# intel-aero/aero-optical-flow

Measured on AMD Instinct MI355X. Metric: frame-pairs/s (640x480, 8x8 SAD, +-4 search), higher is better.
Workload: dtype u8

## Files before the change

aero-optical-flow_amd/csrc/aof_device.hpp:

```cpp
#pragma once

#include <hip/hip_runtime.h>

#include <cstdint>

#include "aof_internal.hpp"

namespace aof {

typedef unsigned long long u64;
typedef uint32_t u32x2 __attribute__((ext_vector_type(2)));
typedef uint32_t u32x4 __attribute__((ext_vector_type(4)));

constexpr int kRawBuffer = 0x00020000;

__device__ __forceinline__ uint32_t fast_div(uint32_t n, FastDiv d) { return (__umulhi(n, d.mul) + n) >> d.shift; }

__device__ __forceinline__ int equalise_delta(const uint32_t *sums, int64_t pair, int level,
                                              uint32_t npix)
{
    if (!sums) return 0;
    const uint32_t sp = sums[pair * 4 + 0 * 2 + level];
    const uint32_t sc = sums[pair * 4 + 1 * 2 + level];
    const int mp = (int)((sp + npix / 2) / npix);
    const int mc = (int)((sc + npix / 2) / npix);
    return mp - mc;
}

__device__ __forceinline__ int clamp_u8(int v) { return v < 0 ? 0 : (v > 255 ? 255 : v); }

typedef unsigned short ushort2_t __attribute__((ext_vector_type(2)));

__device__ __forceinline__ uint32_t sat_delta_u16x2(int delta)
{
    const uint32_t m = (uint32_t)(delta < 0 ? -delta : delta);
    return (m << 8) | (m << 24);
}

template <bool NEG>
__device__ __forceinline__ uint32_t sat_shift_u8x4(uint32_t v, uint32_t d8)
{
    const ushort2_t odd = __builtin_bit_cast(ushort2_t, v), even = __builtin_bit_cast(ushort2_t, v << 8);
    const ushort2_t d = __builtin_bit_cast(ushort2_t, d8);
    const ushort2_t o2 = NEG ? __builtin_elementwise_sub_sat(odd, d) : __builtin_elementwise_add_sat(odd, d);
    const ushort2_t e2 = NEG ? __builtin_elementwise_sub_sat(even, d) : __builtin_elementwise_add_sat(even, d);
    return __builtin_amdgcn_perm(__builtin_bit_cast(uint32_t, o2), __builtin_bit_cast(uint32_t, e2),
                                 0x07030501u);
}

__device__ __forceinline__ uint32_t sat_add_u8x4(uint32_t v, int delta)
{
    const uint32_t d8 = sat_delta_u16x2(delta);
    return delta < 0 ? sat_shift_u8x4<true>(v, d8) : sat_shift_u8x4<false>(v, d8);
}

__device__ __forceinline__ uint4 sat_add_u8x16(uint4 v, int delta)
{
    const uint32_t d8 = sat_delta_u16x2(delta);
    if (delta < 0) {
        v.x = sat_shift_u8x4<true>(v.x, d8); v.y = sat_shift_u8x4<true>(v.y, d8);
        v.z = sat_shift_u8x4<true>(v.z, d8); v.w = sat_shift_u8x4<true>(v.w, d8);
    } else {
        v.x = sat_shift_u8x4<false>(v.x, d8); v.y = sat_shift_u8x4<false>(v.y, d8);
        v.z = sat_shift_u8x4<false>(v.z, d8); v.w = sat_shift_u8x4<false>(v.w, d8);
    }
    return v;
}

__device__ __forceinline__ uint32_t box2(uint32_t a, uint32_t b)
{
    const uint32_t m = 0x00FF00FFu;
    const uint32_t s = (a & m) + ((a >> 8) & m) + (b & m) + ((b >> 8) & m) + 0x00020002u;
    return (s >> 2) & m;
}

__device__ __forceinline__ uint32_t byte_sum(uint32_t w, uint32_t acc)
{
    return __builtin_amdgcn_sad_u8(w, 0u, acc);
}

__device__ __forceinline__ uint32_t wave_min_u32(uint32_t v)
{
#pragma unroll
    for (int o = 32; o >= 1; o >>= 1) {
        const uint32_t other = (uint32_t)__shfl_xor((int)v, o, 64);
        v = other < v ? other : v;
    }
    return v;
}

__device__ __forceinline__ uint32_t wave_sum_u32(uint32_t v)
{
#pragma unroll
    for (int o = 32; o >= 1; o >>= 1) v += (uint32_t)__shfl_xor((int)v, o, 64);
    return v;
}

__device__ __forceinline__ void wave_vote(uint32_t *hist, int bin, bool active)
{
    unsigned long long todo = __ballot(active);
    while (todo) {
        const int leader = __ffsll((long long)todo) - 1;
        const int b = __shfl(bin, leader, 64);
        const unsigned long long same = __ballot(active && bin == b) & todo;
        if ((int)(threadIdx.x & 63) == leader) atomicAdd(&hist[b], (uint32_t)__popcll(same));
        todo &= ~same;
    }
}

__device__ __forceinline__ void wave_vote2(uint32_t *hist_x, uint32_t *hist_y, int bin_x, int bin_y, bool active)
{
    const unsigned long long todo = __ballot(active);
    if (todo == 0) return;
    const int key = bin_x | (bin_y << 16);
    const int leader = __ffsll((long long)todo) - 1;
    const int k = __shfl(key, leader, 64);
    if ((__ballot(active && key == k) & todo) == todo) {
        if ((int)(threadIdx.x & 63) == leader) {
            const uint32_t c = (uint32_t)__popcll(todo);
            atomicAdd(&hist_x[k & 0xFFFF], c);
            atomicAdd(&hist_y[k >> 16], c);
        }
        return;
    }
    wave_vote(hist_x, bin_x, active);
    wave_vote(hist_y, bin_y, active);
}

__device__ __forceinline__ void wave_vote_weighted(uint32_t *hist, int bin, int weight, unsigned long long m1, unsigned long long m2,
                                                   unsigned long long m3, unsigned long long m4)
{
    unsigned long long todo = m1 | m2 | m3 | m4;
    while (todo) {
        const int leader = __ffsll((long long)todo) - 1;
        const int b = __shfl(bin, leader, 64);
        const unsigned long long same = __ballot(weight != 0 && bin == b) & todo;
        const uint32_t total = (uint32_t)(__popcll(same & m1) + 2 * __popcll(same & m2) + 3 * __popcll(same & m3) + 4 * __popcll(same & m4));
        if ((int)(threadIdx.x & 63) == leader) atomicAdd(&hist[b], total);
        todo &= ~same;
    }
}

__device__ __forceinline__ void wave_vote2_weighted(uint32_t *hist_x, uint32_t *hist_y, int key, int weight)
{
    const unsigned long long m1 = __ballot(weight == 1), m2 = __ballot(weight == 2), m3 = __ballot(weight == 3), m4 = __ballot(weight == 4);
    const unsigned long long todo = m1 | m2 | m3 | m4;
    if (todo == 0) return;
    const int leader = __ffsll((long long)todo) - 1;
    const int k = __shfl(key, leader, 64);
    if ((__ballot(weight != 0 && key == k) & todo) == todo) {
        if ((int)(threadIdx.x & 63) == leader) {
            const uint32_t total = (uint32_t)(__popcll(m1) + 2 * __popcll(m2) + 3 * __popcll(m3) + 4 * __popcll(m4));
            atomicAdd(&hist_x[k & 0xFFFF], total);
            atomicAdd(&hist_y[k >> 16], total);
        }
        return;
    }
    wave_vote_weighted(hist_x, key & 0xFFFF, weight, m1, m2, m3, m4);
    wave_vote_weighted(hist_y, key >> 16, weight, m1, m2, m3, m4);
}

__device__ __forceinline__ uint32_t xcd_remap(uint32_t b, uint32_t total)
{
    const uint32_t q = total / 8, r = total % 8, xcd = b % 8, slot = b / 8;
    const uint32_t base = xcd < r ? xcd * (q + 1) : r * (q + 1) + (xcd - r) * q;
    return base + slot;
}

}
```

aero-optical-flow_amd/csrc/aof_reduce.hpp:

```cpp
#pragma once

#include "aof_device.hpp"
#include "aof_internal.hpp"

namespace aof {

__device__ __forceinline__ void peak_window(int pos, int n, int *lo, int *hi)
{
    *lo = *hi = pos;
    if (pos > 1 && pos < n - 2) { *lo = pos - 2; *hi = pos + 2; }
    else if (pos == 0) { *hi = pos + 2; }
    else if (pos == n - 1) { *lo = pos - 2; }
    else if (pos == 1) { *lo = pos - 1; *hi = pos + 2; }
    else if (pos == n - 2) { *lo = pos - 2; *hi = pos + 1; }
}

template <typename T>
__device__ __forceinline__ T floor_div(T a, T b)
{
    T q = a / b;
    if ((a % b) < 0) q--;
    return q;
}

__device__ __forceinline__ void write_flow(const FlowTail &a, int64_t pair, int n, uint32_t vx, uint32_t wx, uint32_t vy,
                                           uint32_t wy, const int *sums)
{
#pragma clang fp contract(off)
    const int centre = 2 * a.range + 1;
    aof_flow out;
    out.flow_x = out.flow_y = 0.0f;
    out.count = (uint32_t)sums[2];
    out.quality = 0;
    out.flags = 0;
    out.pred_x = out.pred_y = 0;
    int px = 0, py = 0;
    const long long count = sums[2];
    const bool small = (long long)n * a.nblocks < (1ll << 28);
    if (count > (long long)a.min_valid && count > 0) {
        if (a.hist_filter) {
            out.flow_x = (__fdiv_rn((float)vx, (float)wx) - (float)centre) / 2.0f;
            out.flow_y = (__fdiv_rn((float)vy, (float)wy) - (float)centre) / 2.0f;
            if (small) {
                px = floor_div<int>((int)(2 * vx + wx), (int)(2 * wx)) - centre;
                py = floor_div<int>((int)(2 * vy + wy), (int)(2 * wy)) - centre;
            } else {
                px = (int)(floor_div<long long>(2ll * vx + wx, 2ll * wx) - centre);
                py = (int)(floor_div<long long>(2ll * vy + wy, 2ll * wy) - centre);
            }
        } else {
            out.flow_x = __fdiv_rn((float)sums[0] * 0.5f, (float)count);
            out.flow_y = __fdiv_rn((float)sums[1] * 0.5f, (float)count);
            if (small) {
                px = floor_div<int>(2 * sums[0] + (int)count, 2 * (int)count);
                py = floor_div<int>(2 * sums[1] + (int)count, 2 * (int)count);
            } else {
                px = (int)floor_div<long long>(2ll * sums[0] + count, 2ll * count);
                py = (int)floor_div<long long>(2ll * sums[1] + count, 2ll * count);
            }
        }
        out.quality = small ? (uint8_t)((uint32_t)count * 255u / (uint32_t)a.nblocks)
                            : (uint8_t)((unsigned long long)count * 255ull / (unsigned long long)a.nblocks);
        out.flags |= AOF_FLAG_FLOW_VALID;
    }
    if (a.emit_predictor) {
        out.pred_x = (int8_t)px;
        out.pred_y = (int8_t)py;
    } else if (a.pred) {
        const aof_flow p = a.pred[pair];
        out.pred_x = p.pred_x;
        out.pred_y = p.pred_y;
        if (p.flags & AOF_FLAG_FLOW_VALID) out.flags |= AOF_FLAG_PRED_VALID;
    }
    a.flows[pair] = out;
}

__device__ __forceinline__ void finalise_flow_wave_bins(const FlowTail &a, int64_t pair, uint32_t hx, uint32_t hy,
                                                        int sum2x, int sum2y, int total, aof_flow *record_out = nullptr,
                                                        const aof_flow *pred_rec = nullptr);

__device__ __forceinline__ void finalise_flow_wave(const FlowTail &a, int64_t pair, const uint32_t *hist_x,
                                                   const uint32_t *hist_y, const int *sums, aof_flow *record_out = nullptr,
                                                   const aof_flow *pred_rec = nullptr)
{
    const int n = 2 * (2 * a.range + 1) + 1;
    const int k = (int)(threadIdx.x & 63);
    finalise_flow_wave_bins(a, pair, k < n ? hist_x[k] : 0u, k < n ? hist_y[k] : 0u, sums[0], sums[1], sums[2],
                            record_out, pred_rec);
}

__device__ __forceinline__ void finalise_flow_wave_bins(const FlowTail &a, int64_t pair, uint32_t hx, uint32_t hy,
                                                        int sum2x, int sum2y, int total, aof_flow *record_out,
                                                        const aof_flow *pred_rec)
{
    const int centre = 2 * a.range + 1, n = 2 * centre + 1;
    const int k = (int)(threadIdx.x & 63);
    const int sums[3] = {sum2x, sum2y, total};
    uint32_t mx = hx, my = hy;
#pragma unroll
    for (int o = 32; o >= 1; o >>= 1) {
        const uint32_t ox = (uint32_t)__shfl_xor((int)mx, o, 64), oy = (uint32_t)__shfl_xor((int)my, o, 64);
        mx = ox > mx ? ox : mx;
        my = oy > my ? oy : my;
    }
    const int posx = __ffsll((long long)__ballot(k < n && hx == mx)) - 1;
    const int posy = __ffsll((long long)__ballot(k < n && hy == my)) - 1;
    int lox, hix, loy, hiy;
    peak_window(posx, n, &lox, &hix);
    peak_window(posy, n, &loy, &hiy);
    const bool inx = k >= lox && k <= hix, iny = k >= loy && k <= hiy;
    const uint32_t vx = wave_sum_u32(inx ? (uint32_t)k * hx : 0u), wx = wave_sum_u32(inx ? hx : 0u);
    const uint32_t vy = wave_sum_u32(iny ? (uint32_t)k * hy : 0u), wy = wave_sum_u32(iny ? hy : 0u);
    const bool axis_y = k == 1;
    const uint32_t v = axis_y ? vy : vx, w = axis_y ? wy : wx;
    const int s2 = axis_y ? sums[1] : sums[0];
    const long long count = sums[2];
    const bool valid = count > (long long)a.min_valid && count > 0;
    const bool small = (long long)n * a.nblocks < (1ll << 28);
    float flow = 0.0f;
    int pred = 0;
    if (k < 2 && valid) {
#pragma clang fp contract(off)
        if (a.hist_filter) {
            flow = (__fdiv_rn((float)v, (float)w) - (float)centre) / 2.0f;
            if (a.emit_predictor)
                pred = small ? floor_div<int>((int)(2 * v + w), (int)(2 * w)) - centre
                             : (int)(floor_div<long long>(2ll * v + w, 2ll * w) - centre);
        } else {
            flow = __fdiv_rn((float)s2 * 0.5f, (float)count);
            if (a.emit_predictor)
                pred = small ? floor_div<int>(2 * s2 + (int)count, 2 * (int)count)
                             : (int)floor_div<long long>(2ll * s2 + count, 2ll * count);
        }
    }
    const float flow_y = __shfl(flow, 1, 64);
    const int pred_y = __shfl(pred, 1, 64);
    if (k == 0) {
        aof_flow out;
        out.flow_x = flow; out.flow_y = flow_y;
        out.count = (uint32_t)sums[2];
        out.quality = 0;
        out.flags = 0;
        out.pred_x = out.pred_y = 0;
        if (valid) {
            out.quality = small ? (uint8_t)((uint32_t)count * 255u / (uint32_t)a.nblocks)
                                : (uint8_t)((unsigned long long)count * 255ull / (unsigned long long)a.nblocks);
            out.flags |= AOF_FLAG_FLOW_VALID;
        }
        if (a.emit_predictor) {
            out.pred_x = (int8_t)pred;
            out.pred_y = (int8_t)pred_y;
        } else if (a.pred) {
            const aof_flow p = pred_rec ? *pred_rec : a.pred[pair];
            out.pred_x = p.pred_x;
            out.pred_y = p.pred_y;
            if (p.flags & AOF_FLAG_FLOW_VALID) out.flags |= AOF_FLAG_PRED_VALID;
        }
        a.flows[pair] = out;
        if (record_out) *record_out = out;
    }
}

__device__ __forceinline__ void vote_add_agent(uint32_t *p, uint32_t v)
{
    (void)__hip_atomic_fetch_add(p, v, __ATOMIC_RELAXED, __HIP_MEMORY_SCOPE_AGENT);
}

__device__ __forceinline__ void wave_vote_agent(uint32_t *hist, int bin, bool active)
{
    unsigned long long todo = __ballot(active);
    while (todo) {
        const int leader = __ffsll((long long)todo) - 1;
        const int b = __shfl(bin, leader, 64);
        const unsigned long long same = __ballot(active && bin == b) & todo;
        if ((int)(threadIdx.x & 63) == leader) vote_add_agent(&hist[b], (uint32_t)__popcll(same));
        todo &= ~same;
    }
}

__device__ __forceinline__ void vote_and_arrive(const VoteMem &vm, int range, uint32_t pair, bool member, bool ok,
                                                int bin_x, int bin_y)
{
    const unsigned long long members = __ballot(member);
    if (members == 0) return;
    const int n = 2 * (2 * range + 1) + 1, lane = (int)(threadIdx.x & 63);
    uint32_t *rec = vm.base + (size_t)pair * vm.stride, *hist_x = rec + 2, *hist_y = rec + 2 + n;
    ok = ok && member;
    const unsigned long long voters = __ballot(ok);
    const int head = __ffsll((long long)members) - 1;
    const unsigned long long arrival = ((unsigned long long)__popcll(members) << 32) | (unsigned long long)__popcll(voters);
    bool one_motion = true;
    int k = 0;
    if (voters) {
        const int key = bin_x | (bin_y << 8);
        k = __builtin_amdgcn_readlane(key, __ffsll((long long)voters) - 1);
        one_motion = (__ballot(ok && key == k) & voters) == voters;
    }
    if (one_motion) {
        if (lane == head) {
            if (voters) {
                const uint32_t c = (uint32_t)__popcll(voters);
                vote_add_agent(&hist_x[k & 0xFF], c);
                vote_add_agent(&hist_y[k >> 8], c);
            }
            (void)__hip_atomic_fetch_add(reinterpret_cast<unsigned long long *>(rec), arrival, __ATOMIC_RELAXED,
                                         __HIP_MEMORY_SCOPE_AGENT);
        }
        return;
    }
    wave_vote_agent(hist_x, bin_x, ok);
    wave_vote_agent(hist_y, bin_y, ok);
    if (lane == head)
        (void)__hip_atomic_fetch_add(reinterpret_cast<unsigned long long *>(rec), arrival, __ATOMIC_RELAXED,
                                     __HIP_MEMORY_SCOPE_AGENT);
}

struct NoWalkVotes {
    __device__ __forceinline__ void init() {}
    __device__ __forceinline__ void flush(const VoteMem &, int, uint32_t) {}
    __device__ __forceinline__ void step(const VoteMem &, int, uint32_t, bool, bool, int, int) {}
};
struct WalkVotes {
    int key;
    uint32_t votes, arrivals;

    __device__ __forceinline__ void init() { key = 0; votes = 0; arrivals = 0; }

    __device__ __forceinline__ void flush(const VoteMem &vm, int range, uint32_t pair)
    {
        if (arrivals == 0) return;
        const int n = 2 * (2 * range + 1) + 1;
        uint32_t *rec = vm.base + (size_t)pair * vm.stride, *hist_x = rec + 2, *hist_y = rec + 2 + n;
        if ((threadIdx.x & 63) == 0) {
            if (votes) {
                vote_add_agent(&hist_x[key & 0xFF], votes);
                vote_add_agent(&hist_y[key >> 8], votes);
            }
            (void)__hip_atomic_fetch_add(reinterpret_cast<unsigned long long *>(rec), ((unsigned long long)arrivals << 32) | votes,
                                         __ATOMIC_RELAXED, __HIP_MEMORY_SCOPE_AGENT);
        }
        votes = 0; arrivals = 0;
    }

    __device__ __forceinline__ void step(const VoteMem &vm, int range, uint32_t pair, bool member, bool ok, int bin_x, int bin_y)
    {
        const unsigned long long members = __ballot(member);
        if (members == 0) return;
        ok = ok && member;
        const unsigned long long voters = __ballot(ok);
        const uint32_t nm = (uint32_t)__popcll(members), nv = (uint32_t)__popcll(voters);
        if (voters == 0) { arrivals = (uint32_t)__builtin_amdgcn_readfirstlane((int)(arrivals + nm)); return; }
        const int mine = bin_x | (bin_y << 8);
        const int k = __builtin_amdgcn_readlane(mine, __ffsll((long long)voters) - 1);
        if ((__ballot(ok && mine == k) & voters) == voters) {
            if (votes != 0 && key != k) flush(vm, range, pair);
            key = k;
            votes = (uint32_t)__builtin_amdgcn_readfirstlane((int)(votes + nv));
            arrivals = (uint32_t)__builtin_amdgcn_readfirstlane((int)(arrivals + nm));
            return;
        }
        flush(vm, range, pair);
        const int n = 2 * (2 * range + 1) + 1;
        uint32_t *rec = vm.base + (size_t)pair * vm.stride;
        wave_vote_agent(rec + 2, bin_x, ok);
        wave_vote_agent(rec + 2 + n, bin_y, ok);
        if ((threadIdx.x & 63) == 0)
            (void)__hip_atomic_fetch_add(reinterpret_cast<unsigned long long *>(rec), ((unsigned long long)nm << 32) | nv, __ATOMIC_RELAXED,
                                         __HIP_MEMORY_SCOPE_AGENT);
    }
};

__device__ __forceinline__ void await_votes_and_finalise(const VoteMem &vm, const FlowTail &tail, uint32_t pair)
{
    const uint64_t deadline_ticks = vm.deadline_ticks;
    const int centre = 2 * tail.range + 1, n = 2 * centre + 1, lane = (int)(threadIdx.x & 63);
    uint32_t *rec = vm.base + (size_t)pair * vm.stride, *hist_x = rec + 2, *hist_y = rec + 2 + n;
    const uint64_t t0 = __builtin_amdgcn_s_memrealtime();
    uint32_t hx = 0, hy = 0;
    int total = 0;
    bool complete = false;
    for (;;) {
        uint32_t arrived = 0, announced = 0;
        if (lane < n) {
            hx = __hip_atomic_load(&hist_x[lane], __ATOMIC_RELAXED, __HIP_MEMORY_SCOPE_AGENT);
            hy = __hip_atomic_load(&hist_y[lane], __ATOMIC_RELAXED, __HIP_MEMORY_SCOPE_AGENT);
        } else if (lane == 63) {
            const unsigned long long a = __hip_atomic_load(reinterpret_cast<unsigned long long *>(rec), __ATOMIC_RELAXED,
                                                           __HIP_MEMORY_SCOPE_AGENT);
            arrived = (uint32_t)(a >> 32);
            announced = (uint32_t)a;
        }
        arrived = (uint32_t)__shfl((int)arrived, 63, 64);
        announced = (uint32_t)__shfl((int)announced, 63, 64);
        total = (int)wave_sum_u32(hx);
        complete = arrived == (uint32_t)tail.nblocks && (uint32_t)total == announced && wave_sum_u32(hy) == announced;
        if (complete || __builtin_amdgcn_s_memrealtime() - t0 > deadline_ticks) break;
        __builtin_amdgcn_s_sleep(8);
    }
    if (lane < n) {
        __hip_atomic_store(&hist_x[lane], 0u, __ATOMIC_RELAXED, __HIP_MEMORY_SCOPE_AGENT);
        __hip_atomic_store(&hist_y[lane], 0u, __ATOMIC_RELAXED, __HIP_MEMORY_SCOPE_AGENT);
    } else if (lane == 63) {
        __hip_atomic_store(reinterpret_cast<unsigned long long *>(rec), 0ull, __ATOMIC_RELAXED, __HIP_MEMORY_SCOPE_AGENT);
    }
    if (!complete) {
        if (lane == 0) {
            aof_flow none;
            __builtin_memset(&none, 0, sizeof(none));
            tail.flows[pair] = none;
            __hip_atomic_store(vm.fault, pair + 1u, __ATOMIC_RELEASE, __HIP_MEMORY_SCOPE_SYSTEM);
        }
        return;
    }
    const int sum2x = (int)wave_sum_u32((uint32_t)((lane - centre) * (int)hx));
    const int sum2y = (int)wave_sum_u32((uint32_t)((lane - centre) * (int)hy));
    finalise_flow_wave_bins(tail, (int64_t)pair, hx, hy, sum2x, sum2y, total);
}

__device__ __forceinline__ void finalise_flow(const FlowTail &a, int64_t pair, const uint32_t *hist_x,
                                              const uint32_t *hist_y, const int *sums)
{
    const int centre = 2 * a.range + 1, n = 2 * centre + 1;
    uint32_t vx = 0, wx = 0, vy = 0, wy = 0;
    if (a.hist_filter && sums[2] > a.min_valid && sums[2] > 0) {
        int posx = 0, posy = 0;
        uint32_t maxx = 0, maxy = 0;
        for (int k = 0; k < n; k++) {
            if (hist_x[k] > maxx) { maxx = hist_x[k]; posx = k; }
            if (hist_y[k] > maxy) { maxy = hist_y[k]; posy = k; }
        }
        int lo, hi;
        peak_window(posx, n, &lo, &hi);
        for (int k = lo; k <= hi; k++) { vx += (uint32_t)k * hist_x[k]; wx += hist_x[k]; }
        peak_window(posy, n, &lo, &hi);
        for (int k = lo; k <= hi; k++) { vy += (uint32_t)k * hist_y[k]; wy += hist_y[k]; }
    }
    write_flow(a, pair, n, vx, wx, vy, wy, sums);
}

}
```

aero-optical-flow_amd/csrc/k_reduce.hip:

```cpp
#include "aof_device.hpp"
#include "aof_internal.hpp"
#include "aof_reduce.hpp"

namespace aof {

namespace {

constexpr int kThreads = 256;
constexpr int kMaxHist = 256;
constexpr int64_t kMidPairs = 1024;
constexpr int64_t kWidePairs = 512;

template <int GROUP, int kThreads = 256>
__global__ __launch_bounds__(kThreads) void k_reduce(ReduceArgs a)
{
    constexpr int kGroups = kThreads / GROUP;
    __shared__ uint32_t s_hist[kGroups][2][kMaxHist];
    __shared__ int s_sums[kGroups][3];
    const int grp = (int)threadIdx.x / GROUP, tid = (int)threadIdx.x % GROUP;
    const int64_t pair = (int64_t)blockIdx.x * kGroups + grp;
    if (GROUP < kThreads && pair >= a.n_pairs) return;
    auto sync = [] { if (GROUP == kThreads) __syncthreads(); else __builtin_amdgcn_wave_barrier(); };
    uint32_t (*hist)[kMaxHist] = s_hist[grp];
    int *sums = s_sums[grp];
    const int centre = 2 * a.tail.range + 1, n = 2 * centre + 1;
    for (int k = tid; k < n; k += GROUP) { hist[0][k] = 0; hist[1][k] = 0; }
    if (tid < 3) sums[tid] = 0;
    sync();

    if (a.parts) {
        const uint32_t *parts = a.parts + (size_t)pair * a.nstrips * (size_t)(2 * n);
        for (int k = tid; k < 2 * n; k += GROUP) {
            uint32_t v = 0;
            for (int st = 0; st < a.nstrips; st++) v += parts[(size_t)st * (2 * n) + k];
            const int axis = k >= n, bin = k - axis * n;
            hist[axis][bin] = v;
            if (v) {
                atomicAdd(&sums[axis], (bin - centre) * (int)v);
                if (!axis) atomicAdd(&sums[2], (int)v);
            }
        }
        sync();
    } else {
    const aof_block *blocks = a.blocks + pair * a.tail.nblocks;
    const uint8_t *subdirs = a.subdirs ? a.subdirs + pair * a.tail.nblocks : nullptr;
    int s2x = 0, s2y = 0, cnt = 0;
    auto vote = [&](bool ok, aof_block r, int sd) {
        ok = ok && !(r.sad == AOF_SAD_SKIPPED || (int)r.sad >= a.value_threshold);
        int hx = 0, hy = 0;
        if (ok && subdirs) {
            hx = (sd == 0 || sd == 1 || sd == 7) ? 1 : ((sd == 3 || sd == 4 || sd == 5) ? -1 : 0);
            hy = (sd == 1 || sd == 2 || sd == 3) ? 1 : ((sd == 5 || sd == 6 || sd == 7) ? -1 : 0);
        }
        const int vx = 2 * r.dx + hx, vy = 2 * r.dy + hy;
        wave_vote2(hist[0], hist[1], vx + centre, vy + centre, ok);
        if (ok) { s2x += vx; s2y += vy; cnt++; }
    };
    typedef uint32_t u32_bytes __attribute__((aligned(1)));
    const uint32_t *words = reinterpret_cast<const uint32_t *>(blocks);
    const int quads = a.tail.nblocks / 4;
    const int qrounds = (quads + GROUP - 1) / GROUP;
    auto vote_quad = [&](bool have, const uint32_t (&w)[4], uint32_t sd4) {
        int key[4], weight = 0, first = 0;
        bool ok[4], messy = false;
#pragma unroll
        for (int j = 0; j < 4; j++) {
            const uint32_t sad = w[j] >> 16;
            ok[j] = have && !(sad == AOF_SAD_SKIPPED || (int)sad >= a.value_threshold);
            const int sd = (int)((sd4 >> (8 * j)) & 0xFFu);
            int hx = 0, hy = 0;
            if (subdirs) {
                hx = (sd == 0 || sd == 1 || sd == 7) ? 1 : ((sd == 3 || sd == 4 || sd == 5) ? -1 : 0);
                hy = (sd == 1 || sd == 2 || sd == 3) ? 1 : ((sd == 5 || sd == 6 || sd == 7) ? -1 : 0);
            }
            const int vx = 2 * (int)(int8_t)(w[j] & 0xFFu) + hx, vy = 2 * (int)(int8_t)((w[j] >> 8) & 0xFFu) + hy;
            key[j] = (vx + centre) | ((vy + centre) << 16);
            if (ok[j]) {
                s2x += vx; s2y += vy; cnt++;
                if (weight == 0) first = key[j];
                else if (key[j] != first) messy = true;
                weight++;
            }
        }
        if (__ballot(messy) == 0) {
            wave_vote2_weighted(hist[0], hist[1], first, weight);
        } else {
#pragma unroll
            for (int j = 0; j < 4; j++) wave_vote2(hist[0], hist[1], key[j] & 0xFFFF, key[j] >> 16, ok[j]);
        }
    };
    constexpr int kBatchQ = 3;
    for (int it0 = 0; it0 < qrounds; it0 += kBatchQ) {
        uint32_t rec[kBatchQ][4], sdir[kBatchQ];
#pragma unroll
        for (int k = 0; k < kBatchQ; k++) {
            const int q = (it0 + k) * GROUP + tid;
#pragma unroll
            for (int j = 0; j < 4; j++) rec[k][j] = 0xFFFF0000u;
            sdir[k] = 0x08080808u;
            if (it0 + k < qrounds && q < quads) {
                __builtin_memcpy(rec[k], words + 4 * q, 16);
                if (subdirs) sdir[k] = *reinterpret_cast<const u32_bytes *>(subdirs + 4 * q);
            }
        }
#pragma unroll
        for (int k = 0; k < kBatchQ; k++) {
            if (it0 + k >= qrounds) break;
            const int q = (it0 + k) * GROUP + tid;
            vote_quad(q < quads, rec[k], sdir[k]);
        }
    }
    {
        const int b = 4 * quads + tid;
        const bool in = b < a.tail.nblocks;
        aof_block r;
        r.dx = 0; r.dy = 0; r.sad = AOF_SAD_SKIPPED;
        if (in) r = blocks[b];
        vote(in, r, in && subdirs ? subdirs[b] : 8);
    }
    s2x = (int)wave_sum_u32((uint32_t)s2x);
    s2y = (int)wave_sum_u32((uint32_t)s2y);
    cnt = (int)wave_sum_u32((uint32_t)cnt);
    if ((tid & 63) == 0) {
        atomicAdd(&sums[0], s2x);
        atomicAdd(&sums[1], s2y);
        atomicAdd(&sums[2], cnt);
    }
    sync();
    }
    if (n <= 64) {
        if (tid < 64) finalise_flow_wave(a.tail, pair, hist[0], hist[1], sums);
    } else if (tid == 0) {
        finalise_flow(a.tail, pair, hist[0], hist[1], sums);
    }
}

__global__ __launch_bounds__(kThreads) void k_reduce_chunk(ReduceArgs a, int chunks)
{
    __shared__ uint32_t hist[2][kMaxHist];
    const int chunk = (int)(blockIdx.x % (uint32_t)chunks);
    const int64_t pair = (int64_t)(blockIdx.x / (uint32_t)chunks);
    const int tid = threadIdx.x;
    const int centre = 2 * a.tail.range + 1, n = 2 * centre + 1;
    for (int k = tid; k < n; k += kThreads) { hist[0][k] = 0; hist[1][k] = 0; }
    __syncthreads();
    const int per = (a.tail.nblocks + chunks - 1) / chunks;
    const int b0 = chunk * per, b1 = min(a.tail.nblocks, b0 + per);
    const uint32_t *blocks = reinterpret_cast<const uint32_t *>(a.blocks) + pair * a.tail.nblocks;
    const uint8_t *subdirs = a.subdirs ? a.subdirs + pair * a.tail.nblocks : nullptr;
    for (int base = b0; base < b1; base += kThreads) {
        const int b = base + tid;
        const bool in = b < b1;
        const aof_block r = __builtin_bit_cast(aof_block, in ? blocks[b] : 0xFFFF0000u);
        const int sd = in && subdirs ? subdirs[b] : 8;
        const bool ok = in && !(r.sad == AOF_SAD_SKIPPED || (int)r.sad >= a.value_threshold);
        int hx = 0, hy = 0;
        if (ok && subdirs) {
            hx = (sd == 0 || sd == 1 || sd == 7) ? 1 : ((sd == 3 || sd == 4 || sd == 5) ? -1 : 0);
            hy = (sd == 1 || sd == 2 || sd == 3) ? 1 : ((sd == 5 || sd == 6 || sd == 7) ? -1 : 0);
        }
        wave_vote(hist[0], 2 * r.dx + hx + centre, ok);
        wave_vote(hist[1], 2 * r.dy + hy + centre, ok);
    }
    __syncthreads();
    uint32_t *out = a.chunk_parts + ((size_t)pair * chunks + chunk) * (size_t)(2 * n);
    for (int k = tid; k < 2 * n; k += kThreads) out[k] = k < n ? hist[0][k] : hist[1][k - n];
}

}

int launch_reduce(const ReduceArgs &a, void *stream)
{
    if (a.n_pairs == 0) return 0;
    if (a.n_pairs > 0x7FFFFFFF) return (int)hipErrorInvalidValue;
    const int chunks = a.parts ? 0 : reduce_chunks(a.tail.nblocks);
    if (chunks > 0 && a.chunk_parts && a.n_pairs * chunks <= 0x7FFFFFFF) {
        hipLaunchKernelGGL(k_reduce_chunk, dim3((uint32_t)(a.n_pairs * chunks)), dim3(kThreads), 0,
                           static_cast<hipStream_t>(stream), a, chunks);
        ReduceArgs b = a;
        b.parts = a.chunk_parts;
        b.nstrips = chunks;
        hipLaunchKernelGGL(k_reduce<kThreads>, dim3((uint32_t)a.n_pairs), dim3(kThreads), 0,
                           static_cast<hipStream_t>(stream), b);
        return (int)hipGetLastError();
    }
    if (a.tail.nblocks <= 256 && !a.parts)
        hipLaunchKernelGGL(k_reduce<64>, dim3((uint32_t)((a.n_pairs + 3) / 4)), dim3(kThreads), 0,
                           static_cast<hipStream_t>(stream), a);
    else if (a.n_pairs <= kWidePairs && a.tail.nblocks >= 2048 && !a.parts)
        hipLaunchKernelGGL((k_reduce<1024, 1024>), dim3((uint32_t)a.n_pairs), dim3(1024), 0,
                           static_cast<hipStream_t>(stream), a);
    else if (a.n_pairs <= kMidPairs && a.tail.nblocks >= 2048 && !a.parts)
        hipLaunchKernelGGL((k_reduce<512, 512>), dim3((uint32_t)a.n_pairs), dim3(512), 0,
                           static_cast<hipStream_t>(stream), a);
    else
        hipLaunchKernelGGL(k_reduce<kThreads>, dim3((uint32_t)a.n_pairs), dim3(kThreads), 0,
                           static_cast<hipStream_t>(stream), a);
    return (int)hipGetLastError();
}

}
```

Measured before the change: 7.917 million.

## Add dense per-pair reduce kernel with DPP wave reductions and uniform-vote fast path

```diff
diff --git a/aero-optical-flow_amd/csrc/aof_device.hpp b/aero-optical-flow_amd/csrc/aof_device.hpp
--- a/aero-optical-flow_amd/csrc/aof_device.hpp
+++ b/aero-optical-flow_amd/csrc/aof_device.hpp
@@ -96,25 +96,73 @@
     return v;
 }
 
+struct CrossLds {
+    static constexpr bool kSpelledOut = true;
+    static __device__ __forceinline__ uint32_t sum(uint32_t v) { return wave_sum_u32(v); }
+    static __device__ __forceinline__ int lane(int v, int from) { return __shfl(v, from, 64); }
+};
+
+template <int kCtrl>
+__device__ __forceinline__ uint32_t dpp_u32(uint32_t v)
+{
+    return (uint32_t)__builtin_amdgcn_update_dpp((int)v, (int)v, kCtrl, 0xF, 0xF, false);
+}
+
+constexpr int kDppXor1 = 0xB1, kDppXor2 = 0x4E, kDppRor4 = 0x124, kDppRor8 = 0x128;
+
+__device__ __forceinline__ uint32_t wave_sum_u32_dpp(uint32_t v)
+{
+    v += dpp_u32<kDppXor1>(v);
+    v += dpp_u32<kDppXor2>(v);
+    v += dpp_u32<kDppRor4>(v);
+    v += dpp_u32<kDppRor8>(v);
+    return (uint32_t)__builtin_amdgcn_readlane((int)v, 0) + (uint32_t)__builtin_amdgcn_readlane((int)v, 16) +
+           (uint32_t)__builtin_amdgcn_readlane((int)v, 32) + (uint32_t)__builtin_amdgcn_readlane((int)v, 48);
+}
+
+__device__ __forceinline__ uint32_t wave_max_u32_dpp(uint32_t v)
+{
+    auto mx = [](uint32_t a, uint32_t b) { return a > b ? a : b; };
+    v = mx(v, dpp_u32<kDppXor1>(v));
+    v = mx(v, dpp_u32<kDppXor2>(v));
+    v = mx(v, dpp_u32<kDppRor4>(v));
+    v = mx(v, dpp_u32<kDppRor8>(v));
+    return mx(mx((uint32_t)__builtin_amdgcn_readlane((int)v, 0), (uint32_t)__builtin_amdgcn_readlane((int)v, 16)),
+              mx((uint32_t)__builtin_amdgcn_readlane((int)v, 32), (uint32_t)__builtin_amdgcn_readlane((int)v, 48)));
+}
+
+struct CrossDpp {
+    static constexpr bool kSpelledOut = false;
+    static __device__ __forceinline__ uint32_t sum(uint32_t v) { return wave_sum_u32_dpp(v); }
+    static __device__ __forceinline__ uint32_t max(uint32_t v) { return wave_max_u32_dpp(v); }
+    static __device__ __forceinline__ int lane(int v, int from) { return __builtin_amdgcn_readlane(v, from); }
+    static __device__ __forceinline__ float lane(float v, int from)
+    {
+        return __builtin_bit_cast(float, __builtin_amdgcn_readlane(__builtin_bit_cast(int, v), from));
+    }
+};
+
+template <class X = CrossLds>
 __device__ __forceinline__ void wave_vote(uint32_t *hist, int bin, bool active)
 {
     unsigned long long todo = __ballot(active);
     while (todo) {
         const int leader = __ffsll((long long)todo) - 1;
-        const int b = __shfl(bin, leader, 64);
+        const int b = X::lane(bin, leader);
         const unsigned long long same = __ballot(active && bin == b) & todo;
         if ((int)(threadIdx.x & 63) == leader) atomicAdd(&hist[b], (uint32_t)__popcll(same));
         todo &= ~same;
     }
 }
 
+template <class X = CrossLds>
 __device__ __forceinline__ void wave_vote2(uint32_t *hist_x, uint32_t *hist_y, int bin_x, int bin_y, bool active)
 {
     const unsigned long long todo = __ballot(active);
     if (todo == 0) return;
     const int key = bin_x | (bin_y << 16);
     const int leader = __ffsll((long long)todo) - 1;
-    const int k = __shfl(key, leader, 64);
+    const int k = X::lane(key, leader);
     if ((__ballot(active && key == k) & todo) == todo) {
         if ((int)(threadIdx.x & 63) == leader) {
             const uint32_t c = (uint32_t)__popcll(todo);
@@ -123,17 +171,18 @@
         }
         return;
     }
-    wave_vote(hist_x, bin_x, active);
-    wave_vote(hist_y, bin_y, active);
-}
-
+    wave_vote<X>(hist_x, bin_x, active);
+    wave_vote<X>(hist_y, bin_y, active);
+}
+
+template <class X = CrossLds>
 __device__ __forceinline__ void wave_vote_weighted(uint32_t *hist, int bin, int weight, unsigned long long m1, unsigned long long m2,
                                                    unsigned long long m3, unsigned long long m4)
 {
     unsigned long long todo = m1 | m2 | m3 | m4;
     while (todo) {
         const int leader = __ffsll((long long)todo) - 1;
-        const int b = __shfl(bin, leader, 64);
+        const int b = X::lane(bin, leader);
         const unsigned long long same = __ballot(weight != 0 && bin == b) & todo;
         const uint32_t total = (uint32_t)(__popcll(same & m1) + 2 * __popcll(same & m2) + 3 * __popcll(same & m3) + 4 * __popcll(same & m4));
         if ((int)(threadIdx.x & 63) == leader) atomicAdd(&hist[b], total);
@@ -141,13 +190,14 @@
     }
 }
 
+template <class X = CrossLds>
 __device__ __forceinline__ void wave_vote2_weighted(uint32_t *hist_x, uint32_t *hist_y, int key, int weight)
 {
     const unsigned long long m1 = __ballot(weight == 1), m2 = __ballot(weight == 2), m3 = __ballot(weight == 3), m4 = __ballot(weight == 4);
     const unsigned long long todo = m1 | m2 | m3 | m4;
     if (todo == 0) return;
     const int leader = __ffsll((long long)todo) - 1;
-    const int k = __shfl(key, leader, 64);
+    const int k = X::lane(key, leader);
     if ((__ballot(weight != 0 && key == k) & todo) == todo) {
         if ((int)(threadIdx.x & 63) == leader) {
             const uint32_t total = (uint32_t)(__popcll(m1) + 2 * __popcll(m2) + 3 * __popcll(m3) + 4 * __popcll(m4));
@@ -156,8 +206,8 @@
         }
         return;
     }
-    wave_vote_weighted(hist_x, key & 0xFFFF, weight, m1, m2, m3, m4);
-    wave_vote_weighted(hist_y, key >> 16, weight, m1, m2, m3, m4);
+    wave_vote_weighted<X>(hist_x, key & 0xFFFF, weight, m1, m2, m3, m4);
+    wave_vote_weighted<X>(hist_y, key >> 16, weight, m1, m2, m3, m4);
 }
 
 __device__ __forceinline__ uint32_t xcd_remap(uint32_t b, uint32_t total)
diff --git a/aero-optical-flow_amd/csrc/aof_reduce.hpp b/aero-optical-flow_amd/csrc/aof_reduce.hpp
--- a/aero-optical-flow_amd/csrc/aof_reduce.hpp
+++ b/aero-optical-flow_amd/csrc/aof_reduce.hpp
@@ -75,6 +75,7 @@
     a.flows[pair] = out;
 }
 
+template <class X = CrossLds>
 __device__ __forceinline__ void finalise_flow_wave_bins(const FlowTail &a, int64_t pair, uint32_t hx, uint32_t hy,
                                                         int sum2x, int sum2y, int total, aof_flow *record_out = nullptr,
                                                         const aof_flow *pred_rec = nullptr);
@@ -89,6 +90,7 @@
                             record_out, pred_rec);
 }
 
+template <class X>
 __device__ __forceinline__ void finalise_flow_wave_bins(const FlowTail &a, int64_t pair, uint32_t hx, uint32_t hy,
                                                         int sum2x, int sum2y, int total, aof_flow *record_out,
                                                         const aof_flow *pred_rec)
@@ -97,11 +99,16 @@
     const int k = (int)(threadIdx.x & 63);
     const int sums[3] = {sum2x, sum2y, total};
     uint32_t mx = hx, my = hy;
+    if constexpr (X::kSpelledOut) {
 #pragma unroll
-    for (int o = 32; o >= 1; o >>= 1) {
-        const uint32_t ox = (uint32_t)__shfl_xor((int)mx, o, 64), oy = (uint32_t)__shfl_xor((int)my, o, 64);
-        mx = ox > mx ? ox : mx;
-        my = oy > my ? oy : my;
+        for (int o = 32; o >= 1; o >>= 1) {
+            const uint32_t ox = (uint32_t)__shfl_xor((int)mx, o, 64), oy = (uint32_t)__shfl_xor((int)my, o, 64);
+            mx = ox > mx ? ox : mx;
+            my = oy > my ? oy : my;
+        }
+    } else {
+        mx = X::max(mx);
+        my = X::max(my);
     }
     const int posx = __ffsll((long long)__ballot(k < n && hx == mx)) - 1;
     const int posy = __ffsll((long long)__ballot(k < n && hy == my)) - 1;
@@ -109,8 +116,8 @@
     peak_window(posx, n, &lox, &hix);
     peak_window(posy, n, &loy, &hiy);
     const bool inx = k >= lox && k <= hix, iny = k >= loy && k <= hiy;
-    const uint32_t vx = wave_sum_u32(inx ? (uint32_t)k * hx : 0u), wx = wave_sum_u32(inx ? hx : 0u);
-    const uint32_t vy = wave_sum_u32(iny ? (uint32_t)k * hy : 0u), wy = wave_sum_u32(iny ? hy : 0u);
+    const uint32_t vx = X::sum(inx ? (uint32_t)k * hx : 0u), wx = X::sum(inx ? hx : 0u);
+    const uint32_t vy = X::sum(iny ? (uint32_t)k * hy : 0u), wy = X::sum(iny ? hy : 0u);
     const bool axis_y = k == 1;
     const uint32_t v = axis_y ? vy : vx, w = axis_y ? wy : wx;
     const int s2 = axis_y ? sums[1] : sums[0];
@@ -133,8 +140,15 @@
                              : (int)floor_div<long long>(2ll * s2 + count, 2ll * count);
         }
     }
-    const float flow_y = __shfl(flow, 1, 64);
-    const int pred_y = __shfl(pred, 1, 64);
+    float flow_y;
+    int pred_y;
+    if constexpr (X::kSpelledOut) {
+        flow_y = __shfl(flow, 1, 64);
+        pred_y = __shfl(pred, 1, 64);
+    } else {
+        flow_y = X::lane(flow, 1);
+        pred_y = X::lane(pred, 1);
+    }
     if (k == 0) {
         aof_flow out;
         out.flow_x = flow; out.flow_y = flow_y;
diff --git a/aero-optical-flow_amd/csrc/k_reduce.hip b/aero-optical-flow_amd/csrc/k_reduce.hip
--- a/aero-optical-flow_amd/csrc/k_reduce.hip
+++ b/aero-optical-flow_amd/csrc/k_reduce.hip
@@ -8,8 +8,6 @@
 
 constexpr int kThreads = 256;
 constexpr int kMaxHist = 256;
-constexpr int64_t kMidPairs = 1024;
-constexpr int64_t kWidePairs = 512;
 
 template <int GROUP, int kThreads = 256>
 __global__ __launch_bounds__(kThreads) void k_reduce(ReduceArgs a)
@@ -28,7 +26,7 @@
     if (tid < 3) sums[tid] = 0;
     sync();
 
-    if (a.parts) {
+    if (GROUP == kThreads || a.parts) {
         const uint32_t *parts = a.parts + (size_t)pair * a.nstrips * (size_t)(2 * n);
         for (int k = tid; k < 2 * n; k += GROUP) {
             uint32_t v = 0;
@@ -132,6 +130,146 @@
         if (tid < 64) finalise_flow_wave(a.tail, pair, hist[0], hist[1], sums);
     } else if (tid == 0) {
         finalise_flow(a.tail, pair, hist[0], hist[1], sums);
+    }
+}
+
+template <int kLanes, int kMaxRounds>
+__global__ __launch_bounds__(kLanes) void k_reduce_dense(ReduceArgs a)
+{
+    using X = CrossDpp;
+    __shared__ uint32_t hist[2][kMaxHist];
+    const int tid = (int)threadIdx.x;
+    const int64_t pair = (int64_t)blockIdx.x;
+    const int centre = 2 * a.tail.range + 1, n = 2 * centre + 1;
+    const int nblocks = a.tail.nblocks;
+    typedef uint32_t u32_bytes __attribute__((aligned(1)));
+    const uint32_t *words = reinterpret_cast<const uint32_t *>(a.blocks) + pair * nblocks;
+    const uint8_t *subdirs = a.subdirs ? a.subdirs + pair * nblocks : nullptr;
+    const int quads = (nblocks + 3) / 4;
+    const int rounds = (quads + kLanes - 1) / kLanes;
+
+    auto load = [&](int r0, uint32_t (&rec)[kMaxRounds][4], uint32_t (&sdir)[kMaxRounds]) {
+#pragma unroll
+        for (int k = 0; k < kMaxRounds; k++) {
+            const int q = (r0 + k) * kLanes + tid;
+#pragma unroll
+            for (int j = 0; j < 4; j++) rec[k][j] = 0xFFFF0000u;
+            sdir[k] = 0x08080808u;
+            if (r0 + k < rounds && q < quads) {
+                const int at = min(4 * q, nblocks - 4);
+                __builtin_memcpy(rec[k], words + at, 16);
+                if (subdirs) sdir[k] = *reinterpret_cast<const u32_bytes *>(subdirs + at);
+            }
+        }
+    };
+    const uint32_t reject = (uint32_t)min(max(a.value_threshold, 0), (int)AOF_SAD_SKIPPED) << 16;
+    auto motion = [&](uint32_t w, uint32_t sd4, int j) { return (w & 0xFFFFu) | (subdirs ? ((sd4 >> (8 * j)) & 0xFFu) << 16 : 0u); };
+    auto bins = [&](uint32_t m) {
+        const int sd = (int)(m >> 16);
+        int hx = 0, hy = 0;
+        if (subdirs) {
+            hx = (sd == 0 || sd == 1 || sd == 7) ? 1 : ((sd == 3 || sd == 4 || sd == 5) ? -1 : 0);
+            hy = (sd == 1 || sd == 2 || sd == 3) ? 1 : ((sd == 5 || sd == 6 || sd == 7) ? -1 : 0);
+        }
+        const int vx = 2 * (int)(int8_t)(m & 0xFFu) + hx, vy = 2 * (int)(int8_t)((m >> 8) & 0xFFu) + hy;
+        return (vx + centre) | ((vy + centre) << 16);
+    };
+    auto vote_quad = [&](const uint32_t (&rec)[4], uint32_t sd4) {
+        int key[4], weight = 0, first = 0;
+        bool ok[4], messy = false;
+#pragma unroll
+        for (int j = 0; j < 4; j++) {
+            ok[j] = rec[j] < reject;
+            key[j] = bins(motion(rec[j], sd4, j));
+            if (ok[j]) {
+                if (weight == 0) first = key[j];
+                else if (key[j] != first) messy = true;
+                weight++;
+            }
+        }
+        if (__ballot(messy) == 0) {
+            wave_vote2_weighted<X>(hist[0], hist[1], first, weight);
+        } else {
+#pragma unroll
+            for (int j = 0; j < 4; j++) wave_vote2<X>(hist[0], hist[1], key[j] & 0xFFFF, key[j] >> 16, ok[j]);
+        }
+    };
+    auto vote = [&](int r0, uint32_t (&rec)[kMaxRounds][4], uint32_t (&sdir)[kMaxRounds]) {
+        const int last = quads - 1, stale = 4 * quads - nblocks;
+        if (stale && last / kLanes >= r0 && last / kLanes < r0 + kMaxRounds && tid == last % kLanes) {
+#pragma unroll
+            for (int k = 0; k < kMaxRounds; k++) {
+                if (r0 + k != last / kLanes) continue;
+#pragma unroll
+                for (int j = 0; j < 3; j++)
+                    if (j < stale) { rec[k][j] = 0xFFFF0000u; sdir[k] = (sdir[k] & ~(0xFFu << (8 * j))) | (8u << (8 * j)); }
+            }
+        }
+        uint32_t lo = 0xFFFFFFFFu, hi = 0u, weight = 0;
+#pragma unroll
+        for (int k = 0; k < kMaxRounds; k++) {
+            if (r0 + k >= rounds) break;
+#pragma unroll
+            for (int j = 0; j < 4; j++) {
+                const bool ok = rec[k][j] < reject;
+                const uint32_t m = motion(rec[k][j], sdir[k], j);
+                lo = min(lo, ok ? m : 0xFFFFFFFFu);
+                hi = max(hi, ok ? m : 0u);
+                weight += ok;
+            }
+        }
+        const unsigned long long voters = __ballot(weight != 0);
+        if (voters == 0) return;
+        const uint32_t m = (uint32_t)X::lane((int)lo, __ffsll((long long)voters) - 1);
+        if (__ballot(weight != 0 && (lo != m || hi != m)) == 0) {
+            const uint32_t total = X::sum(weight);
+            if ((tid & 63) == 0) {
+                const int key = bins(m);
+                atomicAdd(&hist[0][key & 0xFFFF], total);
+                atomicAdd(&hist[1][key >> 16], total);
+            }
+            return;
+        }
+#pragma unroll
+        for (int k = 0; k < kMaxRounds; k++) {
+            if (r0 + k >= rounds) break;
+            vote_quad(rec[k], sdir[k]);
+        }
+    };
+
+    {
+        uint32_t rec[kMaxRounds][4], sdir[kMaxRounds];
+        load(0, rec, sdir);
+        for (int k = tid; k < n; k += kLanes) { hist[0][k] = 0; hist[1][k] = 0; }
+        __syncthreads();
+        vote(0, rec, sdir);
+    }
+    for (int r0 = kMaxRounds; r0 < rounds; r0 += kMaxRounds) {
+        uint32_t rec[kMaxRounds][4], sdir[kMaxRounds];
+        load(r0, rec, sdir);
+        vote(r0, rec, sdir);
+    }
+    __syncthreads();
+    if (tid >= 64) return;
+    if (n <= 64) {
+        const uint32_t hx = tid < n ? hist[0][tid] : 0u, hy = tid < n ? hist[1][tid] : 0u;
+        const int total = (int)X::sum(hx);
+        int s2x = 0, s2y = 0;
+        if (!a.tail.hist_filter) {
+            s2x = (int)X::sum((uint32_t)((tid - centre) * (int)hx));
+            s2y = (int)X::sum((uint32_t)((tid - centre) * (int)hy));
+        }
+        finalise_flow_wave_bins<X>(a.tail, pair, hx, hy, s2x, s2y, total);
+    } else {
+        int s[3] = {0, 0, 0};
+        for (int k = tid; k < n; k += 64) {
+            s[0] += (k - centre) * (int)hist[0][k];
+            s[1] += (k - centre) * (int)hist[1][k];
+            s[2] += (int)hist[0][k];
+        }
+#pragma unroll
+        for (int j = 0; j < 3; j++) s[j] = (int)X::sum((uint32_t)s[j]);
+        if (tid == 0) finalise_flow(a.tail, pair, hist[0], hist[1], s);
     }
 }
 
@@ -184,18 +322,16 @@
                            static_cast<hipStream_t>(stream), b);
         return (int)hipGetLastError();
     }
-    if (a.tail.nblocks <= 256 && !a.parts)
-        hipLaunchKernelGGL(k_reduce<64>, dim3((uint32_t)((a.n_pairs + 3) / 4)), dim3(kThreads), 0,
-                           static_cast<hipStream_t>(stream), a);
-    else if (a.n_pairs <= kWidePairs && a.tail.nblocks >= 2048 && !a.parts)
-        hipLaunchKernelGGL((k_reduce<1024, 1024>), dim3((uint32_t)a.n_pairs), dim3(1024), 0,
-                           static_cast<hipStream_t>(stream), a);
-    else if (a.n_pairs <= kMidPairs && a.tail.nblocks >= 2048 && !a.parts)
-        hipLaunchKernelGGL((k_reduce<512, 512>), dim3((uint32_t)a.n_pairs), dim3(512), 0,
-                           static_cast<hipStream_t>(stream), a);
+    const dim3 per_pair((uint32_t)a.n_pairs);
+    hipStream_t s = static_cast<hipStream_t>(stream);
+    if (a.parts)
+        hipLaunchKernelGGL(k_reduce<kThreads>, per_pair, dim3(kThreads), 0, s, a);
+    else if (a.tail.nblocks <= 256)
+        hipLaunchKernelGGL(k_reduce<64>, dim3((uint32_t)((a.n_pairs + 3) / 4)), dim3(kThreads), 0, s, a);
+    else if (a.tail.nblocks >= 2048)
+        hipLaunchKernelGGL((k_reduce_dense<512, 4>), per_pair, dim3(512), 0, s, a);
     else
-        hipLaunchKernelGGL(k_reduce<kThreads>, dim3((uint32_t)a.n_pairs), dim3(kThreads), 0,
-                           static_cast<hipStream_t>(stream), a);
+        hipLaunchKernelGGL((k_reduce_dense<256, 2>), per_pair, dim3(256), 0, s, a);
     return (int)hipGetLastError();
 }
 
```

After: 8.080 million (median of 6 runs). +2.1%, better.
